# irfanICMLL/structure_knowledge_distillation

Measured on AMD Instinct MI355X. Metric: distillation-step images/sec @512x512 (Pi+Pa+Ho), higher is better.
Workload: dtype f32; 1 GPU; BASELINE configs[2]: ResNet18-PSPNet student + frozen ResNet101-PSPNet teacher, Pi+Pa+Ho (SAGAN D, spectral norm, WGAN-GP), batch 8 per GPU, 512x512, 19 classes; global_batch=8, parallelism=dp1

## Files before the change

structure_knowledge_distillation_amd/csrc/conv1x1.hip:

```cpp
#include <stdio.h>
#include <stdlib.h>

#include "skd_common.hpp"

namespace skd {
namespace {

typedef float f32x16 __attribute__((ext_vector_type(16)));

constexpr int kTM = 128, kTN = 128, kBK = 16, kLDK = kBK + 4, kMinWG = 3;
constexpr int kQK = kBK / 4;
constexpr int kRPP = kThreads / kQK;
constexpr int kRB = kTN / kRPP;
constexpr int kStageFloats = (kTM + kTN) * kLDK;
constexpr size_t kConvLds = sizeof(float) * 2 * kStageFloats;
constexpr int kProMaxK = 512;

__device__ __forceinline__ float inv_std_of(float var, float eps) { return (var != 0.f || eps != 0.f) ? 1.f / sqrtf(var + eps) : 0.f; }

template <int TM>
struct Staging {
  float4 a[TM / kRPP], b[kRB];
};
struct ProParams {
  float4 pm, pi, pg, pb;
};

template <bool PRO, int TM>
__device__ __forceinline__ void stage_load(Staging<TM> &s, const float *__restrict__ X, const float *__restrict__ Wt, int k0,
                                           int gkq, const int64_t (&arow)[TM / kRPP], int64_t wrow0, int K) {
  const float *xa = X + k0 + gkq, *wb = Wt + k0 + gkq;
#pragma unroll
  for (int h = 0; h < TM / kRPP; ++h) s.a[h] = *reinterpret_cast<const float4 *>(xa + arow[h]);
#pragma unroll
  for (int h = 0; h < kRB; ++h) s.b[h] = *reinterpret_cast<const float4 *>(wb + wrow0 + (int64_t)(kRPP * h) * K);
}

__device__ __forceinline__ float pro_one(float x, float m, float is, float g, float b) {
  const float z = __builtin_fmaf((x - m) * is, g, b);
  return z < 0.f ? 0.f : z;
}

template <bool PRO, int TM>
__device__ __forceinline__ void stage_store(const Staging<TM> s, float *stage, int srow, const float *ptab, int K, int kq) {
  constexpr int kRA = TM / kRPP;
  float *sa = stage + srow, *sb = stage + TM * kLDK + srow;
  if (PRO) {
    ProParams pp;
    pp.pm = *reinterpret_cast<const float4 *>(ptab + kq);
    pp.pi = *reinterpret_cast<const float4 *>(ptab + K + kq);
    pp.pg = *reinterpret_cast<const float4 *>(ptab + 2 * K + kq);
    pp.pb = *reinterpret_cast<const float4 *>(ptab + 3 * K + kq);
#pragma unroll
    for (int h = 0; h < kRA; ++h) {
      float4 v = s.a[h];
      v.x = pro_one(v.x, pp.pm.x, pp.pi.x, pp.pg.x, pp.pb.x);
      v.y = pro_one(v.y, pp.pm.y, pp.pi.y, pp.pg.y, pp.pb.y);
      v.z = pro_one(v.z, pp.pm.z, pp.pi.z, pp.pg.z, pp.pb.z);
      v.w = pro_one(v.w, pp.pm.w, pp.pi.w, pp.pg.w, pp.pb.w);
      *reinterpret_cast<float4 *>(sa + kRPP * h * kLDK) = v;
    }
  } else {
#pragma unroll
    for (int h = 0; h < kRA; ++h) *reinterpret_cast<float4 *>(sa + kRPP * h * kLDK) = s.a[h];
  }
#pragma unroll
  for (int h = 0; h < kRB; ++h) *reinterpret_cast<float4 *>(sb + kRPP * h * kLDK) = s.b[h];
}

template <int TM>
__device__ __forceinline__ void tile_mma(const float *stage, f32x16 (&acc)[TM / 64][2]) {
  constexpr int WM = TM / 64;
  const int lane = threadIdx.x & (kWave - 1), wid = threadIdx.x / kWave;
  const int wi = (wid >> 1) * (TM / 2), wj = (wid & 1) * 64;
  const int half = lane >> 5, r = lane & 31;
  const float *pa = stage + (wi + r) * kLDK + half * 4;
  const float *pb = stage + (TM + wj + r) * kLDK + half * 4;
  float4 a[WM], b0 = *reinterpret_cast<const float4 *>(pb), b1 = *reinterpret_cast<const float4 *>(pb + 32 * kLDK);
#pragma unroll
  for (int i = 0; i < WM; ++i) a[i] = *reinterpret_cast<const float4 *>(pa + 32 * i * kLDK);
  __builtin_amdgcn_sched_group_barrier(0x100, WM + 2, 0);
#pragma unroll
  for (int g = 0; g < kBK / 8; ++g) {
    float4 na[WM], nb0 = b0, nb1 = b1;
#pragma unroll
    for (int i = 0; i < WM; ++i) na[i] = a[i];
    if (g + 1 < kBK / 8) {
#pragma unroll
      for (int i = 0; i < WM; ++i) na[i] = *reinterpret_cast<const float4 *>(pa + 32 * i * kLDK + (g + 1) * 8);
      nb0 = *reinterpret_cast<const float4 *>(pb + (g + 1) * 8);
      nb1 = *reinterpret_cast<const float4 *>(pb + 32 * kLDK + (g + 1) * 8);
    }
    const float B0[4] = {b0.x, b0.y, b0.z, b0.w}, B1[4] = {b1.x, b1.y, b1.z, b1.w};
#pragma unroll
    for (int t = 0; t < 4; ++t) {
#pragma unroll
      for (int i = 0; i < WM; ++i) {
        const float av = t == 0 ? a[i].x : t == 1 ? a[i].y : t == 2 ? a[i].z : a[i].w;
        acc[i][0] = __builtin_amdgcn_mfma_f32_32x32x2f32(av, B0[t], acc[i][0], 0, 0, 0);
        acc[i][1] = __builtin_amdgcn_mfma_f32_32x32x2f32(av, B1[t], acc[i][1], 0, 0, 0);
      }
    }
#pragma unroll
    for (int i = 0; i < WM; ++i) a[i] = na[i];
    b0 = nb0; b1 = nb1;
    __builtin_amdgcn_sched_group_barrier(0x008, 2 * WM, 0);
    if (g + 1 < kBK / 8) __builtin_amdgcn_sched_group_barrier(0x100, WM + 2, 0);
    __builtin_amdgcn_sched_group_barrier(0x008, 6 * WM, 0);
  }
}

template <int ACT, bool HAS_RES, bool FULL, bool NT>
__device__ __forceinline__ void store_block(const f32x16 &acc, const float *__restrict__ R, float *__restrict__ Y, int64_t row0,
                                            int col, int64_t M, int N, float mu, float is, float ga, float be, float slope) {
  const int lane = threadIdx.x & (kWave - 1);
  float rv[16];
  int64_t off[16];
#pragma unroll
  for (int q = 0; q < 16; ++q) {
    const int64_t row = row0 + (q & 3) + 8 * (q >> 2) + 4 * (lane >> 5);
    off[q] = row * N + col;
    rv[q] = 0.f;
    if (HAS_RES && (FULL || row < M)) rv[q] = NT ? __builtin_nontemporal_load(R + off[q]) : R[off[q]];
  }
#pragma unroll
  for (int q = 0; q < 16; ++q) {
    const int64_t row = row0 + (q & 3) + 8 * (q >> 2) + 4 * (lane >> 5);
    float z = ((acc[q] - mu) * is) * ga + be;
    if (HAS_RES) z += rv[q];
    if (ACT == SKD_ACT_RELU) z = z < 0.f ? 0.f : z;
    if (ACT == SKD_ACT_LEAKY_RELU) z = z < 0.f ? z * slope : z;
    if (FULL || row < M) {
      if (NT) __builtin_nontemporal_store(z, Y + off[q]);
      else Y[off[q]] = z;
    }
  }
}

template <int TM, int ACT, bool HAS_RES, bool PRO, bool NT>
__device__ __forceinline__ void conv1x1_tile(const float *__restrict__ X, const float *__restrict__ Wt, const float *__restrict__ R,
                                             float *__restrict__ Y, const float *__restrict__ mean, const float *__restrict__ var,
                                             const float *__restrict__ weight, const float *__restrict__ bias,
                                             const float *__restrict__ ppack, float eps, float slope, int64_t M, int K, int N,
                                             int64_t m0, int n0, float *lds) {
  constexpr int WM = TM / 64, kRA = TM / kRPP;
  f32x16 acc[WM][2];
#pragma unroll
  for (int i = 0; i < WM; ++i)
#pragma unroll
    for (int j = 0; j < 2; ++j)
#pragma unroll
      for (int q = 0; q < 16; ++q) acc[i][j][q] = 0.f;
  const int nk = K / kBK;
  const int gt = threadIdx.x, grow = gt / kQK, gkq = (gt % kQK) * 4;
  const int srow = grow * kLDK + gkq;
  int64_t arow[kRA];
#pragma unroll
  for (int h = 0; h < kRA; ++h) {
    const int64_t m = m0 + grow + kRPP * h;
    arow[h] = (m > M - 1 ? M - 1 : m) * K;
  }
  const int64_t wrow0 = (int64_t)(n0 + grow) * K;
  float *ptab = lds + 2 * kStageFloats;
  if (PRO) {
    for (int i = gt * 4; i < 4 * K; i += kThreads * 4) *reinterpret_cast<float4 *>(ptab + i) = *reinterpret_cast<const float4 *>(ppack + i);
    __syncthreads();
  }
  Staging<TM> st;
  stage_load<PRO, TM>(st, X, Wt, 0, gkq, arow, wrow0, K);
  stage_store<PRO, TM>(st, lds, srow, ptab, K, gkq);
  __syncthreads();
  int stage = 0;
  for (int kt = 0; kt < nk; ++kt) {
    const bool more = kt + 1 < nk;
    if (more) stage_load<PRO, TM>(st, X, Wt, (kt + 1) * kBK, gkq, arow, wrow0, K);
    tile_mma<TM>(lds + stage * kStageFloats, acc);
    if (more) stage_store<PRO, TM>(st, lds + (stage ^ 1) * kStageFloats, srow, ptab, K, (kt + 1) * kBK + gkq);
    __syncthreads();
    stage ^= 1;
  }
  const int lane = threadIdx.x & (kWave - 1), wid = threadIdx.x / kWave;
  const int wi = (wid >> 1) * (TM / 2), wj = (wid & 1) * 64;
  const bool full = m0 + TM <= M;
#pragma unroll
  for (int bj = 0; bj < 2; ++bj) {
    const int col = n0 + wj + bj * 32 + (lane & 31);
    const float mu = mean[col], is = inv_std_of(var[col], eps);
    const float ga = weight != nullptr ? fabsf(weight[col]) + eps : 1.f;
    const float be = bias != nullptr ? bias[col] : 0.f;
#pragma unroll
    for (int bi = 0; bi < WM; ++bi) {
      const int64_t row0 = m0 + wi + bi * 32;
      if (full)
        store_block<ACT, HAS_RES, true, NT>(acc[bi][bj], R, Y, row0, col, M, N, mu, is, ga, be, slope);
      else
        store_block<ACT, HAS_RES, false, NT>(acc[bi][bj], R, Y, row0, col, M, N, mu, is, ga, be, slope);
    }
  }
}

template <int ACT, bool HAS_RES, bool PRO, bool NT>
__global__ __launch_bounds__(kThreads, kMinWG) void conv1x1_abn_kernel(
    const float *__restrict__ X, const float *__restrict__ Wt, const float *__restrict__ R, float *__restrict__ Y,
    const float *__restrict__ mean, const float *__restrict__ var, const float *__restrict__ weight,
    const float *__restrict__ bias, const float *__restrict__ ppack, float eps, float slope, int64_t M, int K, int N,
    int tiles_n, int pm, int ct, int p_full) {
  extern __shared__ __attribute__((aligned(16))) float lds[];
  const int xcd = blockIdx.x & 7, j = blockIdx.x >> 3;
  const int per_group = pm * tiles_n;
  const int group = j / per_group, r = j - group * per_group;
  const int per_chunk = pm * ct;
  const int chunk = r / per_chunk, r2 = r - chunk * per_chunk;
  const int pl = r2 / ct;
  const int tn = chunk * ct + (r2 - pl * ct);
  const int64_t tm = ((int64_t)group * pm + pl) * 8 + xcd;
  if (tn >= tiles_n) return;
  const int n0 = tn * kTN;
  if (tm < p_full) {
    const int64_t m0 = tm * kTM;
    if (m0 >= M) return;
    conv1x1_tile<kTM, ACT, HAS_RES, PRO, NT>(X, Wt, R, Y, mean, var, weight, bias, ppack, eps, slope, M, K, N, m0, n0, lds);
  } else {
    const int64_t m0 = (int64_t)p_full * kTM + (tm - p_full) * (kTM / 2);
    if (m0 >= M) return;
    conv1x1_tile<kTM / 2, ACT, HAS_RES, PRO, NT>(X, Wt, R, Y, mean, var, weight, bias, ppack, eps, slope, M, K, N, m0, n0, lds);
  }
}

__global__ void pack_eval_params_kernel(int K, const float *__restrict__ mean, const float *__restrict__ var,
                                        const float *__restrict__ weight, const float *__restrict__ bias, float eps,
                                        float *__restrict__ pack) {
  const int k = blockIdx.x * blockDim.x + threadIdx.x;
  if (k >= K) return;
  pack[k] = mean[k];
  pack[K + k] = inv_std_of(var[k], eps);
  pack[2 * (int64_t)K + k] = weight != nullptr ? fabsf(weight[k]) + eps : 1.f;
  pack[3 * (int64_t)K + k] = bias != nullptr ? bias[k] : 0.f;
}

template <int ACT, bool HAS_RES, bool PRO, bool NT = false>
static int launch(const float *X, const float *Wt, const float *R, float *Y, const float *mean, const float *var,
                  const float *weight, const float *bias, const float *ppack, float eps, float slope, int64_t M, int K, int N,
                  hipStream_t st) {
  static PerDeviceFlag ready;
  bool *rdy = ready.get();
  if (rdy == nullptr) return 0;
  if (!*rdy) {
    if (hipFuncSetAttribute(reinterpret_cast<const void *>(conv1x1_abn_kernel<ACT, HAS_RES, PRO, NT>),
                            hipFuncAttributeMaxDynamicSharedMemorySize, (int)(kConvLds + sizeof(float) * 4 * kProMaxK)) != hipSuccess) return 0;
    *rdy = true;
  }
  const size_t lds_bytes = kConvLds + (PRO ? sizeof(float) * 4 * (size_t)K : 0);
  const int tiles_n = N / kTN;
  const int64_t tiles_m = cdiv(M, kTM);
  const int64_t tile_bytes = (int64_t)kTN * K * sizeof(float);
  int ct = (int)((1 << 20) / tile_bytes), pm = (int)((2 << 20) / tile_bytes);
  if (ct < 1) ct = 1;
  if (pm < 1) pm = 1;
  if (ct >= tiles_n) { ct = tiles_n; pm = 1; }
  else if (!NT) return launch<ACT, HAS_RES, PRO, true>(X, Wt, R, Y, mean, var, weight, bias, ppack, eps, slope, M, K, N, st);
  while (tiles_n % ct) --ct;
  int64_t p_full = tiles_m, panels = tiles_m;
  {
    static PerDeviceFlag cu_known;
    static int cus[64] = {};
    bool *known = cu_known.get();
    int dev = 0;
    if (known != nullptr && hipGetDevice(&dev) == hipSuccess && dev >= 0 && dev < 64) {
      if (!*known) {
        int n = 0;
        if (hipDeviceGetAttribute(&n, hipDeviceAttributeMultiprocessorCount, dev) == hipSuccess && n > 0) cus[dev] = n;
        *known = true;
      }
      const int64_t slots = (int64_t)kMinWG * cus[dev];
      const int64_t tiles = tiles_m * tiles_n;
      if (slots > 0 && tiles > slots && tiles % slots != 0) {
        p_full = (tiles / slots) * slots / tiles_n / 8 * 8;
        const int64_t rest_rows = M - p_full * kTM;
        panels = p_full + cdiv(rest_rows, kTM / 2);
      }
    }
  }
  const int64_t panels_per_xcd = cdiv(cdiv(panels, 8), pm) * pm;
  if (panels_per_xcd * 8 * tiles_n > 2147483647) return 0;
  const int64_t grid = panels_per_xcd * 8 * tiles_n;
  conv1x1_abn_kernel<ACT, HAS_RES, PRO, NT><<<dim3((unsigned)grid), dim3(kThreads), lds_bytes, st>>>(
      X, Wt, R, Y, mean, var, weight, bias, ppack, eps, slope, M, K, N, tiles_n, pm, ct, (int)p_full);
  return ok();
}

}
}

using namespace skd;

extern "C" {

int skd_conv1x1_abn_supported(int64_t M, int K, int N) { return M > 0 && K > 0 && N > 0 && K % kBK == 0 && N % kTN == 0; }

static int conv1x1_dispatch(int64_t M, int K, int N, const float *x, const float *w, const float *residual, float *out,
                            const float *mean, const float *var, const float *weight, const float *bias, const float *ppack,
                            float eps, int activation, float slope, skd_stream_t stream) {
  if (!skd_conv1x1_abn_supported(M, K, N) || !x || !w || !out || !mean || !var) return 0;
  if ((reinterpret_cast<uintptr_t>(x) | reinterpret_cast<uintptr_t>(w) | reinterpret_cast<uintptr_t>(ppack)) & 15) return 0;
  hipStream_t st = as_stream(stream);
#define SKD_C11(A)                                                                                                        \
  if (ppack != nullptr)                                                                                                   \
    return residual ? launch<A, true, true>(x, w, residual, out, mean, var, weight, bias, ppack, eps, slope, M, K, N, st)   \
                    : launch<A, false, true>(x, w, residual, out, mean, var, weight, bias, ppack, eps, slope, M, K, N, st); \
  return residual ? launch<A, true, false>(x, w, residual, out, mean, var, weight, bias, nullptr, eps, slope, M, K, N, st) \
                  : launch<A, false, false>(x, w, residual, out, mean, var, weight, bias, nullptr, eps, slope, M, K, N, st)
  switch (activation) {
    case SKD_ACT_NONE: SKD_C11(SKD_ACT_NONE);
    case SKD_ACT_RELU: SKD_C11(SKD_ACT_RELU);
    case SKD_ACT_LEAKY_RELU: SKD_C11(SKD_ACT_LEAKY_RELU);
    default: return 0;
  }
#undef SKD_C11
}

int skd_conv1x1_abn_nhwc(int64_t M, int K, int N, const float *x, const float *w, const float *residual, float *out,
                         const float *mean, const float *var, const float *weight, const float *bias, float eps,
                         int activation, float slope, skd_stream_t stream) {
  return conv1x1_dispatch(M, K, N, x, w, residual, out, mean, var, weight, bias, nullptr, eps, activation, slope, stream);
}

int skd_abn_pack_eval_params(int K, const float *mean, const float *var, const float *weight, const float *bias, float eps,
                             float *pack, skd_stream_t stream) {
  if (K <= 0 || !mean || !var || !pack) return 0;
  pack_eval_params_kernel<<<dim3((unsigned)cdiv(K, 256)), dim3(256), 0, as_stream(stream)>>>(K, mean, var, weight, bias, eps, pack);
  return ok();
}

int skd_conv1x1_abn_pro_nhwc(int64_t M, int K, int N, const float *x, const float *w, const float *residual, float *out,
                             const float *mean, const float *var, const float *weight, const float *bias, float eps,
                             const float *ppack, int activation, float slope, skd_stream_t stream) {
  if (!ppack || K > kProMaxK) return 0;
  return conv1x1_dispatch(M, K, N, x, w, residual, out, mean, var, weight, bias, ppack, eps, activation, slope, stream);
}

}
```

Baseline: 128.5 images/sec.

## Emulate fp32 1x1 conv GEMM with split-bf16 triple-plane MFMA

Operands are split into three bf16 planes (hi, mid, lo) when staged into LDS, using a swizzled chunk layout. The inner product then uses six bf16 32x32x16 MFMAs per tile instead of the f32 32x32x2 MFMA chain, which keeps close to fp32 accuracy while using the much faster bf16 matrix path. The cost is extra conversion ALU work at staging, a larger LDS footprint, and dropped low-order cross terms, so results are only approximately fp32. CU-count lookup is also reworked to use the stream's device with an atomic cache.

```diff
diff --git a/structure_knowledge_distillation_amd/csrc/conv1x1.hip b/structure_knowledge_distillation_amd/csrc/conv1x1.hip
--- a/structure_knowledge_distillation_amd/csrc/conv1x1.hip
+++ b/structure_knowledge_distillation_amd/csrc/conv1x1.hip
@@ -1,19 +1,26 @@
 #include <stdio.h>
 #include <stdlib.h>
 
+#include <atomic>
+
 #include "skd_common.hpp"
 
 namespace skd {
 namespace {
 
 typedef float f32x16 __attribute__((ext_vector_type(16)));
-
-constexpr int kTM = 128, kTN = 128, kBK = 16, kLDK = kBK + 4, kMinWG = 3;
+typedef __bf16 bf16x8 __attribute__((ext_vector_type(8)));
+typedef __bf16 bf16x2 __attribute__((ext_vector_type(2)));
+typedef float f32x2 __attribute__((ext_vector_type(2)));
+
+constexpr int kTM = 128, kTN = 128, kBK = 16, kMinWG = 3;
 constexpr int kQK = kBK / 4;
 constexpr int kRPP = kThreads / kQK;
 constexpr int kRB = kTN / kRPP;
-constexpr int kStageFloats = (kTM + kTN) * kLDK;
-constexpr size_t kConvLds = sizeof(float) * 2 * kStageFloats;
+constexpr int kPlaneChunks = 2 * 128;
+constexpr int kOperandChunks = 3 * kPlaneChunks;
+constexpr int kStageChunks = 2 * kOperandChunks;
+constexpr size_t kConvLds = sizeof(uint4) * 2 * kStageChunks;
 constexpr int kProMaxK = 512;
 
 __device__ __forceinline__ float inv_std_of(float var, float eps) { return (var != 0.f || eps != 0.f) ? 1.f / sqrtf(var + eps) : 0.f; }
@@ -41,10 +48,32 @@
   return z < 0.f ? 0.f : z;
 }
 
+__device__ __forceinline__ uint32_t pack_bf16(float x, float y) {
+  const f32x2 v = {x, y};
+  return __builtin_bit_cast(uint32_t, __builtin_convertvector(v, bf16x2));
+}
+__device__ __forceinline__ float bf16_lo(uint32_t u) { return __uint_as_float(u << 16); }
+__device__ __forceinline__ float bf16_hi(uint32_t u) { return __uint_as_float(u & 0xffff0000u); }
+
+__device__ __forceinline__ void split_store(float4 v, uint2 *dst) {
+  uint2 p0, p1, p2;
+  p0.x = pack_bf16(v.x, v.y);
+  p0.y = pack_bf16(v.z, v.w);
+  v.x -= bf16_lo(p0.x); v.y -= bf16_hi(p0.x); v.z -= bf16_lo(p0.y); v.w -= bf16_hi(p0.y);
+  p1.x = pack_bf16(v.x, v.y);
+  p1.y = pack_bf16(v.z, v.w);
+  v.x -= bf16_lo(p1.x); v.y -= bf16_hi(p1.x); v.z -= bf16_lo(p1.y); v.w -= bf16_hi(p1.y);
+  p2.x = pack_bf16(v.x, v.y);
+  p2.y = pack_bf16(v.z, v.w);
+  dst[0] = p0;
+  dst[2 * kPlaneChunks] = p1;
+  dst[4 * kPlaneChunks] = p2;
+}
+
 template <bool PRO, int TM>
-__device__ __forceinline__ void stage_store(const Staging<TM> s, float *stage, int srow, const float *ptab, int K, int kq) {
+__device__ __forceinline__ void stage_store(const Staging<TM> s, uint4 *stage, int srow, const float *ptab, int K, int kq) {
   constexpr int kRA = TM / kRPP;
-  float *sa = stage + srow, *sb = stage + TM * kLDK + srow;
+  uint2 *sa = reinterpret_cast<uint2 *>(stage) + srow, *sb = reinterpret_cast<uint2 *>(stage + kOperandChunks) + srow;
   if (PRO) {
     ProParams pp;
     pp.pm = *reinterpret_cast<const float4 *>(ptab + kq);
@@ -58,56 +87,40 @@
       v.y = pro_one(v.y, pp.pm.y, pp.pi.y, pp.pg.y, pp.pb.y);
       v.z = pro_one(v.z, pp.pm.z, pp.pi.z, pp.pg.z, pp.pb.z);
       v.w = pro_one(v.w, pp.pm.w, pp.pi.w, pp.pg.w, pp.pb.w);
-      *reinterpret_cast<float4 *>(sa + kRPP * h * kLDK) = v;
+      split_store(v, sa + 2 * kRPP * h);
     }
   } else {
 #pragma unroll
-    for (int h = 0; h < kRA; ++h) *reinterpret_cast<float4 *>(sa + kRPP * h * kLDK) = s.a[h];
-  }
-#pragma unroll
-  for (int h = 0; h < kRB; ++h) *reinterpret_cast<float4 *>(sb + kRPP * h * kLDK) = s.b[h];
+    for (int h = 0; h < kRA; ++h) split_store(s.a[h], sa + 2 * kRPP * h);
+  }
+#pragma unroll
+  for (int h = 0; h < kRB; ++h) split_store(s.b[h], sb + 2 * kRPP * h);
 }
 
 template <int TM>
-__device__ __forceinline__ void tile_mma(const float *stage, f32x16 (&acc)[TM / 64][2]) {
+__device__ __forceinline__ void tile_mma(const uint4 *stage, f32x16 (&acc)[TM / 64][2]) {
   constexpr int WM = TM / 64;
   const int lane = threadIdx.x & (kWave - 1), wid = threadIdx.x / kWave;
   const int wi = (wid >> 1) * (TM / 2), wj = (wid & 1) * 64;
   const int half = lane >> 5, r = lane & 31;
-  const float *pa = stage + (wi + r) * kLDK + half * 4;
-  const float *pb = stage + (TM + wj + r) * kLDK + half * 4;
-  float4 a[WM], b0 = *reinterpret_cast<const float4 *>(pb), b1 = *reinterpret_cast<const float4 *>(pb + 32 * kLDK);
-#pragma unroll
-  for (int i = 0; i < WM; ++i) a[i] = *reinterpret_cast<const float4 *>(pa + 32 * i * kLDK);
-  __builtin_amdgcn_sched_group_barrier(0x100, WM + 2, 0);
-#pragma unroll
-  for (int g = 0; g < kBK / 8; ++g) {
-    float4 na[WM], nb0 = b0, nb1 = b1;
-#pragma unroll
-    for (int i = 0; i < WM; ++i) na[i] = a[i];
-    if (g + 1 < kBK / 8) {
-#pragma unroll
-      for (int i = 0; i < WM; ++i) na[i] = *reinterpret_cast<const float4 *>(pa + 32 * i * kLDK + (g + 1) * 8);
-      nb0 = *reinterpret_cast<const float4 *>(pb + (g + 1) * 8);
-      nb1 = *reinterpret_cast<const float4 *>(pb + 32 * kLDK + (g + 1) * 8);
-    }
-    const float B0[4] = {b0.x, b0.y, b0.z, b0.w}, B1[4] = {b1.x, b1.y, b1.z, b1.w};
-#pragma unroll
-    for (int t = 0; t < 4; ++t) {
-#pragma unroll
-      for (int i = 0; i < WM; ++i) {
-        const float av = t == 0 ? a[i].x : t == 1 ? a[i].y : t == 2 ? a[i].z : a[i].w;
-        acc[i][0] = __builtin_amdgcn_mfma_f32_32x32x2f32(av, B0[t], acc[i][0], 0, 0, 0);
-        acc[i][1] = __builtin_amdgcn_mfma_f32_32x32x2f32(av, B1[t], acc[i][1], 0, 0, 0);
-      }
-    }
-#pragma unroll
-    for (int i = 0; i < WM; ++i) a[i] = na[i];
-    b0 = nb0; b1 = nb1;
-    __builtin_amdgcn_sched_group_barrier(0x008, 2 * WM, 0);
-    if (g + 1 < kBK / 8) __builtin_amdgcn_sched_group_barrier(0x100, WM + 2, 0);
-    __builtin_amdgcn_sched_group_barrier(0x008, 6 * WM, 0);
-  }
+  const uint4 *pa = stage + half * 128 + ((wi + r) ^ (half * 4));
+  const uint4 *pb = stage + kOperandChunks + half * 128 + ((wj + r) ^ (half * 4));
+  bf16x8 a[WM][3], b[2][3];
+#pragma unroll
+  for (int p = 0; p < 3; ++p) {
+#pragma unroll
+    for (int i = 0; i < WM; ++i) a[i][p] = __builtin_bit_cast(bf16x8, pa[p * kPlaneChunks + 32 * i]);
+#pragma unroll
+    for (int j = 0; j < 2; ++j) b[j][p] = __builtin_bit_cast(bf16x8, pb[p * kPlaneChunks + 32 * j]);
+  }
+  constexpr int kPA[6] = {0, 1, 2, 0, 1, 0}, kPB[6] = {2, 1, 0, 1, 0, 0};
+#pragma unroll
+  for (int t = 0; t < 6; ++t)
+#pragma unroll
+    for (int i = 0; i < WM; ++i)
+#pragma unroll
+      for (int j = 0; j < 2; ++j)
+        acc[i][j] = __builtin_amdgcn_mfma_f32_32x32x16_bf16(a[i][kPA[t]], b[j][kPB[t]], acc[i][j], 0, 0, 0);
 }
 
 template <int ACT, bool HAS_RES, bool FULL, bool NT>
@@ -142,7 +155,7 @@
                                              float *__restrict__ Y, const float *__restrict__ mean, const float *__restrict__ var,
                                              const float *__restrict__ weight, const float *__restrict__ bias,
                                              const float *__restrict__ ppack, float eps, float slope, int64_t M, int K, int N,
-                                             int64_t m0, int n0, float *lds) {
+                                             int64_t m0, int n0, uint4 *lds) {
   constexpr int WM = TM / 64, kRA = TM / kRPP;
   f32x16 acc[WM][2];
 #pragma unroll
@@ -153,7 +166,8 @@
       for (int q = 0; q < 16; ++q) acc[i][j][q] = 0.f;
   const int nk = K / kBK;
   const int gt = threadIdx.x, grow = gt / kQK, gkq = (gt % kQK) * 4;
-  const int srow = grow * kLDK + gkq;
+  const int kh = gkq >> 3;
+  const int srow = 2 * (kh * 128 + (grow ^ (kh * 4))) + ((gkq >> 2) & 1);
   int64_t arow[kRA];
 #pragma unroll
   for (int h = 0; h < kRA; ++h) {
@@ -161,7 +175,7 @@
     arow[h] = (m > M - 1 ? M - 1 : m) * K;
   }
   const int64_t wrow0 = (int64_t)(n0 + grow) * K;
-  float *ptab = lds + 2 * kStageFloats;
+  float *ptab = reinterpret_cast<float *>(lds + 2 * kStageChunks);
   if (PRO) {
     for (int i = gt * 4; i < 4 * K; i += kThreads * 4) *reinterpret_cast<float4 *>(ptab + i) = *reinterpret_cast<const float4 *>(ppack + i);
     __syncthreads();
@@ -174,8 +188,8 @@
   for (int kt = 0; kt < nk; ++kt) {
     const bool more = kt + 1 < nk;
     if (more) stage_load<PRO, TM>(st, X, Wt, (kt + 1) * kBK, gkq, arow, wrow0, K);
-    tile_mma<TM>(lds + stage * kStageFloats, acc);
-    if (more) stage_store<PRO, TM>(st, lds + (stage ^ 1) * kStageFloats, srow, ptab, K, (kt + 1) * kBK + gkq);
+    tile_mma<TM>(lds + stage * kStageChunks, acc);
+    if (more) stage_store<PRO, TM>(st, lds + (stage ^ 1) * kStageChunks, srow, ptab, K, (kt + 1) * kBK + gkq);
     __syncthreads();
     stage ^= 1;
   }
@@ -205,7 +219,7 @@
     const float *__restrict__ mean, const float *__restrict__ var, const float *__restrict__ weight,
     const float *__restrict__ bias, const float *__restrict__ ppack, float eps, float slope, int64_t M, int K, int N,
     int tiles_n, int pm, int ct, int p_full) {
-  extern __shared__ __attribute__((aligned(16))) float lds[];
+  extern __shared__ __attribute__((aligned(16))) uint4 lds[];
   const int xcd = blockIdx.x & 7, j = blockIdx.x >> 3;
   const int per_group = pm * tiles_n;
   const int group = j / per_group, r = j - group * per_group;
@@ -238,6 +252,20 @@
   pack[3 * (int64_t)K + k] = bias != nullptr ? bias[k] : 0.f;
 }
 
+static int cu_count(hipStream_t st) {
+  static std::atomic<int> cus[64];
+  int dev = -1;
+  if (hipStreamGetDevice(st, &dev) != hipSuccess) {
+    (void)hipGetLastError();
+    if (hipGetDevice(&dev) != hipSuccess) return 0;
+  }
+  if (dev < 0 || dev >= 64) return 0;
+  int n = cus[dev].load(std::memory_order_relaxed);
+  if (n == 0 && hipDeviceGetAttribute(&n, hipDeviceAttributeMultiprocessorCount, dev) == hipSuccess && n > 0)
+    cus[dev].store(n, std::memory_order_relaxed);
+  return n > 0 ? n : 0;
+}
+
 template <int ACT, bool HAS_RES, bool PRO, bool NT = false>
 static int launch(const float *X, const float *Wt, const float *R, float *Y, const float *mean, const float *var,
                   const float *weight, const float *bias, const float *ppack, float eps, float slope, int64_t M, int K, int N,
@@ -262,23 +290,12 @@
   while (tiles_n % ct) --ct;
   int64_t p_full = tiles_m, panels = tiles_m;
   {
-    static PerDeviceFlag cu_known;
-    static int cus[64] = {};
-    bool *known = cu_known.get();
-    int dev = 0;
-    if (known != nullptr && hipGetDevice(&dev) == hipSuccess && dev >= 0 && dev < 64) {
-      if (!*known) {
-        int n = 0;
-        if (hipDeviceGetAttribute(&n, hipDeviceAttributeMultiprocessorCount, dev) == hipSuccess && n > 0) cus[dev] = n;
-        *known = true;
-      }
-      const int64_t slots = (int64_t)kMinWG * cus[dev];
-      const int64_t tiles = tiles_m * tiles_n;
-      if (slots > 0 && tiles > slots && tiles % slots != 0) {
-        p_full = (tiles / slots) * slots / tiles_n / 8 * 8;
-        const int64_t rest_rows = M - p_full * kTM;
-        panels = p_full + cdiv(rest_rows, kTM / 2);
-      }
+    const int64_t slots = (int64_t)kMinWG * cu_count(st);
+    const int64_t tiles = tiles_m * tiles_n;
+    if (slots > 0 && tiles > slots && tiles % slots != 0) {
+      p_full = (tiles / slots) * slots / tiles_n / 8 * 8;
+      const int64_t rest_rows = M - p_full * kTM;
+      panels = p_full + cdiv(rest_rows, kTM / 2);
     }
   }
   const int64_t panels_per_xcd = cdiv(cdiv(panels, 8), pm) * pm;
```

Result: faster. 132.1 images/sec, median of 6 (+2.8%).
